# player4771/YOLO-DBL

Hardware: AMD Instinct MI355X
Metric: images/sec @640×640 bs=32 (1/2/4/8 GPU) + mAP@0.5 vs CPU ref (higher is better)
Workload: dtype fp16; 1 GPU; YOLO-DBL-n 640x640 bs=32/GPU fp16 forward+decode+NMS (conf .25, iou .7, max_det 300); model=yolov13n_DBL, global_batch=32, imgsz=640, nc=3, parallelism=dp1, streams_per_gpu=2

## Files before the change

### yolo-dbl_amd/csrc/conv.hip

```cpp
#include <stdlib.h>

#include "conv_common.hpp"

namespace ydbl {

template <bool Q8>
__device__ __forceinline__ int swz(int row, int kv) {
  if constexpr (Q8) return row * 4 + (kv ^ (((row >> 3) & 1) << 1));
  else return row * 4 + (kv ^ (((row >> 2) & 1) << 1));
}

template <typename T, int BM, int BN, int WM, int WN, bool POINTWISE, bool Q8, int PF = 1, int KA = ACT_RT>
__global__ __launch_bounds__(256) void conv_igemm_kernel(ConvArgs<T> p) {
  constexpr int VEC = Vec<T>::N;
  constexpr int BK = 4 * VEC;
  constexpr int TM = BM / WM / 16, TN = BN / WN / 16;
  static_assert(WM * WN == 4 && TM >= 1 && TN >= 1, "tile config");
  static_assert(PF >= 1 && PF <= 4, "prefetch depth");
  constexpr int A_IT = (BN * 4 + 255) / 256, B_IT = (BM * 4 + 255) / 256;
  using vec = typename Vec<T>::type;
  using opv = typename Op<T, Q8>::lds;
  __shared__ opv sA[2][BN * 4];
  __shared__ opv sB[2][BM * 4];

  const int tid = threadIdx.x;
  const int lane = tid & 63, wave = tid >> 6;
  const int g = lane >> 4, r16 = lane & 15;
  const int wm = wave % WM, wn = wave / WM;
  int mb, nb;
  xcd_tile2(mb, nb);
  const int m0 = mb * BM;
  const int n0 = nb * BN;
  __shared__ __align__(16) float s_bias[BN];
  BiasStage<BN> bst;
  bst.fetch(p.bias, n0, p.Cout);

  int64_t arow[A_IT];
  bool aval[A_IT];
#pragma unroll
  for (int it = 0; it < A_IT; ++it) {
    const int v = tid + it * 256;
    const int co = n0 + (v >> 2);
    aval[it] = v < BN * 4 && co < p.Cout;
    arow[it] = (int64_t)(aval[it] ? co : 0) * p.KPAD + (v & 3) * VEC;
  }
  int bb[B_IT], biy[B_IT], bix[B_IT];
  int64_t bpix[B_IT];
  bool bval[B_IT];
#pragma unroll
  for (int it = 0; it < B_IT; ++it) {
    const int v = tid + it * 256;
    int pp = m0 + (v >> 2);
    bval[it] = v < BM * 4 && pp < p.P;
    pp = bval[it] ? pp : 0;
    bpix[it] = pp;
    const int ox = pp % p.Wo;
    const int t = pp / p.Wo;
    const int oy = t % p.Ho;
    bb[it] = t / p.Ho;
    biy[it] = oy * p.S - p.PAD;
    bix[it] = ox * p.S - p.PAD;
  }
  opv ra[PF][A_IT];
  vec rb[PF][B_IT];
  bool rok[PF][B_IT], aok[PF][A_IT];
  int cur_ci = (tid & 3) * VEC, cur_kx = 0, cur_ky = 0;
  if constexpr (!POINTWISE) {
    const int tap = cur_ci / p.Cin;
    cur_ci -= tap * p.Cin;
    cur_ky = tap / p.KW;
    cur_kx = tap - cur_ky * p.KW;
  }
  auto advance = [&]() {
    if constexpr (!POINTWISE) {
      cur_ci += BK;
      while (cur_ci >= p.Cin) {
        cur_ci -= p.Cin;
        if (++cur_kx == p.KW) { cur_kx = 0; ++cur_ky; }
      }
    }
  };
  auto load_step = [&](int ks, opv (&a)[A_IT], bool (&aok)[A_IT], vec (&b)[B_IT], bool (&bok)[B_IT]) {
#pragma unroll
    for (int it = 0; it < A_IT; ++it) {
      aok[it] = aval[it] && ks * BK < p.KPAD;
      a[it] = load_wop_raw<T, Q8>(p.w, arow[it] + ks * BK, aok[it]);
    }
#pragma unroll
    for (int it = 0; it < B_IT; ++it) {
      const int v = tid + it * 256;
      const int k = ks * BK + (v & 3) * VEC;
      const bool kin = k < p.K;
      if constexpr (POINTWISE) {
        bok[it] = bval[it] && kin;
        b[it] = vload_clamped(p.x + bpix[it] * p.xcs + k, p.x, bok[it]);
      } else {
        const int iy = biy[it] + cur_ky * p.DIL, ix = bix[it] + cur_kx * p.DIL;
        bok[it] = bval[it] && kin && iy >= 0 && iy < p.H && ix >= 0 && ix < p.W;
        b[it] = vload_clamped(p.x + ((int64_t)(bb[it] * p.H + iy) * p.W + ix) * p.xcs + cur_ci, p.x, bok[it]);
      }
    }
    advance();
  };
  auto store_step = [&](int buf, const opv (&a)[A_IT], const bool (&aok)[A_IT], const vec (&b)[B_IT],
                        const bool (&bok)[B_IT]) {
#pragma unroll
    for (int it = 0; it < A_IT; ++it) {
      const int v = tid + it * 256;
      if (v < BN * 4) sA[buf][swz<Q8>(v >> 2, v & 3)] = vsel(a[it], aok[it]);
    }
#pragma unroll
    for (int it = 0; it < B_IT; ++it) {
      const int v = tid + it * 256;
      if (v < BM * 4) sB[buf][swz<Q8>(v >> 2, v & 3)] = to_op<T, Q8>(vsel(b[it], bok[it]), p.qs);
    }
  };

  f32x4 acc[TN][TM];
#pragma unroll
  for (int i = 0; i < TN; ++i)
#pragma unroll
    for (int j = 0; j < TM; ++j) acc[i][j] = f32x4{0.f, 0.f, 0.f, 0.f};

  const int nsteps = (p.K + BK - 1) / BK;
#pragma unroll
  for (int u = 0; u < PF; ++u) load_step(u, ra[u], aok[u], rb[u], rok[u]);
  store_step(0, ra[0], aok[0], rb[0], rok[0]);
  bst.commit(s_bias);
  __syncthreads();
  for (int k0 = 0; k0 < nsteps; k0 += PF) {
#pragma unroll
    for (int u = 0; u < PF; ++u) {
      const int ks = k0 + u;
      if (PF > 1 || ks + PF < nsteps) load_step(ks + PF, ra[u], aok[u], rb[u], rok[u]);
      if (ks < nsteps) {
        const int buf = ks & 1;
        opv af[TN], bf[TM];
#pragma unroll
        for (int i = 0; i < TN; ++i) af[i] = sA[buf][swz<Q8>(wn * TN * 16 + i * 16 + r16, g)];
#pragma unroll
        for (int j = 0; j < TM; ++j) bf[j] = sB[buf][swz<Q8>(wm * TM * 16 + j * 16 + r16, g)];
#pragma unroll
        for (int i = 0; i < TN; ++i)
#pragma unroll
          for (int j = 0; j < TM; ++j) acc[i][j] = mfma_op<T, Q8>(af[i], bf[j], acc[i][j]);
        const int nx = (u + 1) % PF;
        if (ks + 1 < nsteps) store_step(buf ^ 1, ra[nx], aok[nx], rb[nx], rok[nx]);
        __syncthreads();
      }
    }
  }

  int64_t pp[TM];
  bool pv[TM];
  int co[TN];
#pragma unroll
  for (int j = 0; j < TM; ++j) {
    pp[j] = m0 + wm * TM * 16 + j * 16 + r16;
    pv[j] = pp[j] < p.P;
  }
#pragma unroll
  for (int i = 0; i < TN; ++i) co[i] = n0 + wn * TN * 16 + i * 16 + 4 * g;
  conv_epilogue<T, TN, TM, Q8, KA>(p, acc, pp, pv, co, s_bias, n0);
}

template <int CV>
__device__ __forceinline__ int tswz(int pix, int cv) {
  if constexpr (CV == 1) return pix;
  else return pix * CV + (cv ^ ((pix / (16 / CV)) & (CV - 1)));
}

template <typename T, int CIN, int S, int TH, int TW, int NTN, int KA = ACT_RT>
__global__ __launch_bounds__(256) void conv3x3_tile_kernel(ConvArgs<T> p, int tiles_x, int tiles_y) {
  constexpr int VEC = Vec<T>::N;
  constexpr int CV = CIN / VEC;
  constexpr int IH = (TH - 1) * S + 3, IW = (TW - 1) * S + 3;
  constexpr int K = 9 * CIN;
  constexpr int BK = 4 * VEC;
  constexpr int KPAD = (K + 31) / 32 * 32;
  constexpr int NSTEP = (K + BK - 1) / BK;
  constexpr int WROW = KPAD / VEC + 1;
  constexpr int TM = TH * TW / 64;
  using vec = typename Vec<T>::type;
  __shared__ vec sx[IH * IW * CV];
  __shared__ vec sw[NTN * 16 * WROW];

  const int tid = threadIdx.x;
  int bid = xcd_remap(blockIdx.x, gridDim.x);
  const int tx = bid % tiles_x; bid /= tiles_x;
  const int ty = bid % tiles_y;
  const int b = bid / tiles_y;
  const int oy0 = ty * TH, ox0 = tx * TW;
  const int iy0 = oy0 * S - p.PAD, ix0 = ox0 * S - p.PAD;
  __shared__ __align__(16) float s_bias[NTN * 16];
  BiasStage<NTN * 16> bst;
  bst.fetch(p.bias, 0, p.Cout);
  {
    constexpr int TOT = IH * IW * CV;
    for (int base = 0; base < TOT; base += 4 * 256) {
      vec t[4];
#pragma unroll
      for (int u = 0; u < 4; ++u) {
        const int i = min(base + u * 256 + tid, TOT - 1);
        const int pix = i / CV, cv = i - pix * CV;
        const int iy = iy0 + pix / IW, ix = ix0 + pix % IW;
        const bool ok = iy >= 0 && iy < p.H && ix >= 0 && ix < p.W;
        t[u] = vload_sel(p.x + ((int64_t)(b * p.H + iy) * p.W + ix) * p.xcs + cv * VEC, p.x, ok);
      }
#pragma unroll
      for (int u = 0; u < 4; ++u) {
        const int i = base + u * 256 + tid;
        if (i < TOT) sx[tswz<CV>(i / CV, i % CV)] = t[u];
      }
    }
    constexpr int WTOT = NTN * 16 * (KPAD / VEC);
    for (int base = 0; base < WTOT; base += 4 * 256) {
      vec t[4];
#pragma unroll
      for (int u = 0; u < 4; ++u) {
        const int i = min(base + u * 256 + tid, WTOT - 1);
        const int co = i / (KPAD / VEC), kv = i % (KPAD / VEC);
        t[u] = vload_sel(p.w + (int64_t)co * p.KPAD + kv * VEC, p.w, co < p.Cout);
      }
#pragma unroll
      for (int u = 0; u < 4; ++u) {
        const int i = base + u * 256 + tid;
        if (i < WTOT) sw[(i / (KPAD / VEC)) * WROW + i % (KPAD / VEC)] = t[u];
      }
    }
  }
  bst.commit(s_bias);
  __syncthreads();

  const int lane = tid & 63, wave = tid >> 6;
  const int g = lane >> 4, r16 = lane & 15;
  int lbase[TM];
#pragma unroll
  for (int j = 0; j < TM; ++j) {
    const int op = wave * TM * 16 + j * 16 + r16;
    const int py = op / TW, px = op % TW;
    lbase[j] = (py * S) * IW + px * S;
  }
  f32x4 acc[NTN][TM];
#pragma unroll
  for (int i = 0; i < NTN; ++i)
#pragma unroll
    for (int j = 0; j < TM; ++j) acc[i][j] = f32x4{0.f, 0.f, 0.f, 0.f};
#pragma unroll
  for (int ks = 0; ks < NSTEP; ++ks) {
    const int k = ks * BK + g * VEC;
    const bool kin = k < K;
    const int tap = kin ? k / CIN : 0, cv = kin ? (k % CIN) / VEC : 0;
    const int ky = tap / 3, kx = tap % 3;
    const int toff = ky * IW + kx;
    vec af[NTN], bf[TM];
#pragma unroll
    for (int i = 0; i < NTN; ++i) af[i] = sw[(i * 16 + r16) * WROW + ks * 4 + g];
#pragma unroll
    for (int j = 0; j < TM; ++j) bf[j] = sx[tswz<CV>(lbase[j] + toff, cv)];
#pragma unroll
    for (int i = 0; i < NTN; ++i)
#pragma unroll
      for (int j = 0; j < TM; ++j) acc[i][j] = mfma_chunk<T>(af[i], bf[j], acc[i][j]);
  }

  int64_t pp[TM];
  bool pv[TM];
  int co[NTN];
#pragma unroll
  for (int j = 0; j < TM; ++j) {
    const int op = wave * TM * 16 + j * 16 + r16;
    const int oy = oy0 + op / TW, ox = ox0 + op % TW;
    pv[j] = oy < p.Ho && ox < p.Wo;
    pp[j] = ((int64_t)b * p.Ho + oy) * p.Wo + ox;
  }
#pragma unroll
  for (int i = 0; i < NTN; ++i) co[i] = i * 16 + 4 * g;
  conv_epilogue<T, NTN, TM, false, KA>(p, acc, pp, pv, co, s_bias, 0);
}

template <typename T, int CIN, int S, int TH, int TW, int NTN>
static void launch_tile(const ConvArgs<T>& a, hipStream_t s) {
  const int tiles_x = (int)cdiv(a.Wo, TW), tiles_y = (int)cdiv(a.Ho, TH);
  const unsigned grid = (unsigned)(a.N * tiles_y * tiles_x);
  if constexpr (sizeof(T) == 2) {
    const int form = epi_host_form(a);
    if (form == YDBL_ACT_SILU)
      return conv3x3_tile_kernel<T, CIN, S, TH, TW, NTN, YDBL_ACT_SILU><<<grid, 256, 0, s>>>(a, tiles_x, tiles_y);
    if (form == YDBL_ACT_NONE)
      return conv3x3_tile_kernel<T, CIN, S, TH, TW, NTN, YDBL_ACT_NONE><<<grid, 256, 0, s>>>(a, tiles_x, tiles_y);
  }
  conv3x3_tile_kernel<T, CIN, S, TH, TW, NTN, ACT_RT><<<grid, 256, 0, s>>>(a, tiles_x, tiles_y);
}

template <typename T, int CIN, int NTN>
static void launch_tile_s(const ConvArgs<T>& a, hipStream_t s) {
  if (a.S == 1) launch_tile<T, CIN, 1, 8, 32, NTN>(a, s);
  else launch_tile<T, CIN, 2, 8, 16, NTN>(a, s);
}

template <typename T, int CIN>
static bool tile_ntn(const ConvArgs<T>& a, hipStream_t s) {
  switch ((a.Cout + 15) / 16) {
    case 1: launch_tile_s<T, CIN, 1>(a, s); return true;
    case 2: launch_tile_s<T, CIN, 2>(a, s); return true;
    case 3: launch_tile_s<T, CIN, 3>(a, s); return true;
    case 4: launch_tile_s<T, CIN, 4>(a, s); return true;
    default: return false;
  }
}

template <typename T>
static bool try_tile(const ConvArgs<T>& a, int kh, hipStream_t s) {
  if (kh != 3 || a.KW != 3 || a.DIL != 1 || a.PAD != 1 || a.Cout > 64 || a.Cout % 4) return false;
  if (a.S != 1 && a.S != 2) return false;
  if ((int64_t)a.Ho * a.Wo < 4096) return false;
  if (a.xcs % Vec<T>::N) return false;
  switch (a.Cin) {
    case 8: return tile_ntn<T, 8>(a, s);
    case 16: return tile_ntn<T, 16>(a, s);
    case 32: return tile_ntn<T, 32>(a, s);
    default: return false;
  }
}

template <typename T, int BM, int BN, bool POINTWISE, bool Q8, int PF = 1, bool SPLIT = false>
__global__ __launch_bounds__(256) void conv_wsk_kernel(ConvArgs<T> p) {
  constexpr int VEC = Vec<T>::N;
  constexpr int BK = 4 * VEC;
  constexpr int BKB = 4 * BK;
  constexpr int TM = BM / 16, TN = BN / 16;
  constexpr int A_IT = BN * 16 / 256, B_IT = BM * 16 / 256;
  static_assert(A_IT >= 1 && B_IT >= 1, "tile");
  using vec = typename Vec<T>::type;
  using opv = typename Op<T, Q8>::lds;
  constexpr int STAGE = 2 * (BN + BM) * 16 * (int)sizeof(opv);
  constexpr int RED = 4 * TN * TM * 64 * 16;
  __shared__ f32x4 smem[(STAGE > RED ? STAGE : RED) / 16];
  opv* sA = reinterpret_cast<opv*>(smem);
  opv* sB = sA + 2 * BN * 16;

  const int tid = threadIdx.x;
  const int lane = tid & 63, wave = tid >> 6;
  const int g = lane >> 4, r16 = lane & 15;
  int mb, nb;
  xcd_tile2(mb, nb);
  const int m0 = mb * BM, n0 = nb * BN;
  const int kv = tid & 15;

  int64_t arow[A_IT];
  bool aval[A_IT];
#pragma unroll
  for (int it = 0; it < A_IT; ++it) {
    const int co = n0 + ((tid + it * 256) >> 4);
    aval[it] = co < p.Cout;
    arow[it] = (int64_t)(aval[it] ? co : 0) * p.KPAD + kv * VEC;
  }
  int bb[B_IT], biy[B_IT], bix[B_IT];
  int64_t bpix[B_IT];
  bool bval[B_IT];
#pragma unroll
  for (int it = 0; it < B_IT; ++it) {
    int pp = m0 + ((tid + it * 256) >> 4);
    bval[it] = pp < p.P;
    pp = bval[it] ? pp : 0;
    bpix[it] = pp;
    const int ox = pp % p.Wo;
    const int t = pp / p.Wo;
    bb[it] = t / p.Ho;
    biy[it] = (t % p.Ho) * p.S - p.PAD;
    bix[it] = ox * p.S - p.PAD;
  }
  const int nsteps_all = (p.K + BKB - 1) / BKB;
  const int z = SPLIT ? (int)blockIdx.z : 0;
  const int s0 = SPLIT ? (int)((int64_t)z * nsteps_all / p.ksplit) : 0;
  const int s1 = SPLIT ? (int)((int64_t)(z + 1) * nsteps_all / p.ksplit) : nsteps_all;
  int cur_ci = s0 * BKB + kv * VEC, cur_kx = 0, cur_ky = 0;
  if constexpr (!POINTWISE) {
    const int tap = cur_ci / p.Cin;
    cur_ci -= tap * p.Cin;
    cur_ky = tap / p.KW;
    cur_kx = tap - cur_ky * p.KW;
  }
  opv ra[PF][A_IT];
  vec rb[PF][B_IT];
  bool aok[PF], bok[PF][B_IT];
  auto load_step = [&](int kb, opv (&a)[A_IT], bool& ak, vec (&b)[B_IT], bool (&bk)[B_IT]) {
    const int k = kb * BKB + kv * VEC;
    const bool kin = k < p.K;
    ak = kin;
#pragma unroll
    for (int it = 0; it < A_IT; ++it) a[it] = load_wop_raw<T, Q8>(p.w, arow[it] + kb * BKB, aval[it] && kin);
#pragma unroll
    for (int it = 0; it < B_IT; ++it) {
      if constexpr (POINTWISE) {
        bk[it] = bval[it] && kin;
        b[it] = vload_clamped(p.x + bpix[it] * p.xcs + k, p.x, bk[it]);
      } else {
        const int iy = biy[it] + cur_ky * p.DIL, ix = bix[it] + cur_kx * p.DIL;
        bk[it] = bval[it] && kin && iy >= 0 && iy < p.H && ix >= 0 && ix < p.W;
        b[it] = vload_clamped(p.x + ((int64_t)(bb[it] * p.H + iy) * p.W + ix) * p.xcs + cur_ci, p.x, bk[it]);
      }
    }
    if constexpr (!POINTWISE) {
      cur_ci += BKB;
      while (cur_ci >= p.Cin) {
        cur_ci -= p.Cin;
        if (++cur_kx == p.KW) { cur_kx = 0; ++cur_ky; }
      }
    }
  };
  auto store_step = [&](int buf, const opv (&a)[A_IT], bool ak, const vec (&b)[B_IT], const bool (&bk)[B_IT]) {
#pragma unroll
    for (int it = 0; it < A_IT; ++it) {
      const int row = (tid + it * 256) >> 4;
      sA[buf * BN * 16 + row * 16 + (kv ^ (row & 15))] = vsel(a[it], aval[it] && ak);
    }
#pragma unroll
    for (int it = 0; it < B_IT; ++it) {
      const int row = (tid + it * 256) >> 4;
      sB[buf * BM * 16 + row * 16 + (kv ^ (row & 15))] = to_op<T, Q8>(vsel(b[it], bk[it]), p.qs);
    }
  };

  f32x4 acc[TN][TM];
#pragma unroll
  for (int i = 0; i < TN; ++i)
#pragma unroll
    for (int j = 0; j < TM; ++j) acc[i][j] = f32x4{0.f, 0.f, 0.f, 0.f};

  const int nsteps = s1 - s0;
#pragma unroll
  for (int u = 0; u < PF; ++u) load_step(s0 + u, ra[u], aok[u], rb[u], bok[u]);
  store_step(0, ra[0], aok[0], rb[0], bok[0]);
  __syncthreads();
  const int myk = wave * 4 + g;
  for (int k0 = 0; k0 < nsteps; k0 += PF) {
#pragma unroll
    for (int u = 0; u < PF; ++u) {
      const int kb = k0 + u;
      if (PF > 1 || kb + PF < nsteps) load_step(s0 + kb + PF, ra[u], aok[u], rb[u], bok[u]);
      if (kb < nsteps) {
        const int buf = kb & 1;
        opv af[TN], bf[TM];
#pragma unroll
        for (int i = 0; i < TN; ++i) {
          const int row = i * 16 + r16;
          af[i] = sA[buf * BN * 16 + row * 16 + (myk ^ (row & 15))];
        }
#pragma unroll
        for (int j = 0; j < TM; ++j) {
          const int row = j * 16 + r16;
          bf[j] = sB[buf * BM * 16 + row * 16 + (myk ^ (row & 15))];
        }
#pragma unroll
        for (int i = 0; i < TN; ++i)
#pragma unroll
          for (int j = 0; j < TM; ++j) acc[i][j] = mfma_op<T, Q8>(af[i], bf[j], acc[i][j]);
        const int nx = (u + 1) % PF;
        if (kb + 1 < nsteps) store_step(buf ^ 1, ra[nx], aok[nx], rb[nx], bok[nx]);
        __syncthreads();
      }
    }
  }

  f32x4* red = reinterpret_cast<f32x4*>(smem);
#pragma unroll
  for (int i = 0; i < TN; ++i)
#pragma unroll
    for (int j = 0; j < TM; ++j) red[((wave * TN + i) * TM + j) * 64 + lane] = acc[i][j];
  __syncthreads();
  for (int t = wave; t < TN * TM; t += 4) {
    const int i = t / TM, j = t % TM;
    f32x4 sum = red[((0 * TN + i) * TM + j) * 64 + lane];
#pragma unroll
    for (int w = 1; w < 4; ++w) {
      const f32x4 o = red[((w * TN + i) * TM + j) * 64 + lane];
      sum = f32x4{sum[0] + o[0], sum[1] + o[1], sum[2] + o[2], sum[3] + o[3]};
    }
    const f32x4 one[1][1] = {{sum}};
    const int64_t pp[1] = {m0 + j * 16 + r16};
    const bool pv[1] = {pp[0] < p.P};
    const int co[1] = {n0 + i * 16 + 4 * g};
    if constexpr (SPLIT) {
      if (pv[0] && co[0] < p.Cout)
        *reinterpret_cast<f32x4*>(p.ws + ((int64_t)z * p.P + pp[0]) * ((p.Cout + 3) & ~3) + co[0]) = sum;
    } else {
      conv_epilogue<T, 1, 1, Q8>(p, one, pp, pv, co);
    }
  }
}

template <typename T, bool Q8>
__global__ __launch_bounds__(256) void splitk_epilogue_kernel(ConvArgs<T> p) {
  const int c4 = (p.Cout + 3) >> 2, cs = c4 * 4;
  const int64_t t = (int64_t)blockIdx.x * 256 + threadIdx.x;
  const int64_t pix = t / c4;
  const int co = (int)(t - pix * c4) * 4;
  const bool ok = pix < p.P;
  const int64_t pc = ok ? pix : 0;
  f32x4 v[4];
#pragma unroll
  for (int z = 0; z < 4; ++z)
    v[z] = z < p.ksplit ? *reinterpret_cast<const f32x4*>(p.ws + ((int64_t)z * p.P + pc) * cs + co) : f32x4{0.f, 0.f, 0.f, 0.f};
  f32x4 sum = v[0];
#pragma unroll
  for (int z = 1; z < 4; ++z)
    if (z < p.ksplit) sum = f32x4{sum[0] + v[z][0], sum[1] + v[z][1], sum[2] + v[z][2], sum[3] + v[z][3]};
  const f32x4 one[1][1] = {{sum}};
  const int64_t pp[1] = {pix};
  const bool pv[1] = {ok};
  const int cc[1] = {co};
  conv_epilogue<T, 1, 1, Q8>(p, one, pp, pv, cc);
}

template <typename T, bool Q8>
void launch_splitk_epilogue(const ConvArgs<T>& a, hipStream_t s) {
  splitk_epilogue_kernel<T, Q8><<<(unsigned)cdiv((int64_t)a.P * ((a.Cout + 3) >> 2), 256), 256, 0, s>>>(a);
}
template void launch_splitk_epilogue<_Float16, false>(const ConvArgs<_Float16>&, hipStream_t);
template void launch_splitk_epilogue<_Float16, true>(const ConvArgs<_Float16>&, hipStream_t);
template void launch_splitk_epilogue<float, false>(const ConvArgs<float>&, hipStream_t);

constexpr int WSK_SPLIT_BELOW = 768;
template <typename T>
static int wsk_ksplit(const ConvArgs<T>& a, int bm, int bn) {
  const char* e = getenv("YDBL_SPLITK");
  if (sizeof(T) != 2 || (e && *e == '0')) return 1;
  const int64_t tiles = cdiv(a.P, bm) * cdiv(a.Cout, bn);
  const int nsteps = (int)cdiv(a.K, 16 * Vec<T>::N);
  if (tiles >= WSK_SPLIT_BELOW || nsteps < 16) return 1;
  int k = (int)std::min<int64_t>(4, (WSK_SPLIT_BELOW + tiles - 1) / tiles);
  while (k > 1 && nsteps / k < 8) --k;
  return k;
}
template <typename T>
static int64_t wsk_ws_bytes(const ConvArgs<T>& a, int ksplit) {
  return ksplit > 1 ? (int64_t)ksplit * a.P * ((a.Cout + 3) & ~3) * 4 : 0;
}

constexpr int WSK_PF = 2;

template <typename T, bool Q8, int BM, int BN>
static void launch_wsk(const ConvArgs<T>& a0, bool pointwise, hipStream_t s) {
  ConvArgs<T> a = a0;
  a.ksplit = wsk_ksplit(a, BM, BN);
  if (a.ksplit > 1 && (!a.ws || a.ws_bytes < wsk_ws_bytes(a, a.ksplit))) a.ksplit = 1;
  dim3 grid((unsigned)cdiv(a.P, BM), (unsigned)cdiv(a.Cout, BN), (unsigned)a.ksplit);
  if (a.ksplit > 1) {
    if (pointwise) conv_wsk_kernel<T, BM, BN, true, Q8, WSK_PF, true><<<grid, 256, 0, s>>>(a);
    else conv_wsk_kernel<T, BM, BN, false, Q8, WSK_PF, true><<<grid, 256, 0, s>>>(a);
    launch_splitk_epilogue<T, Q8>(a, s);
  } else if (pointwise) {
    conv_wsk_kernel<T, BM, BN, true, Q8, WSK_PF><<<grid, 256, 0, s>>>(a);
  } else {
    conv_wsk_kernel<T, BM, BN, false, Q8, WSK_PF><<<grid, 256, 0, s>>>(a);
  }
}

template <typename T>
static void wsk_tiles(const ConvArgs<T>& a, int& bm, int& bn) {
  auto blocks = [&](int m, int n) { return cdiv(a.P, m) * cdiv(a.Cout, n); };
  const int64_t want = 768;
  const char* eh = getenv("YDBL_WSK_HALF");
  if (a.Cout <= 128 && blocks(32, a.Cout <= 64 ? 64 : 128) < 256 && !(eh && *eh == '0')) {
    bm = a.Cout <= 64 ? 16 : 32;
    bn = 64;
    return;
  }
  if (a.Cout <= 32) { bm = blocks(128, 32) >= want ? 128 : 64; bn = 32; return; }
  if (a.Cout <= 64) { bm = blocks(64, 64) >= want ? 64 : 32; bn = 64; return; }
  bm = 32;
  bn = blocks(32, 128) >= want || a.Cout % 128 == 0 ? 128 : 64;
}

template <typename T>
static bool wsk_applies(const ConvArgs<T>& a) { return a.K >= 1024 || (a.K >= 512 && a.P <= 16384); }

template <typename T, bool Q8>
static bool try_wsk(const ConvArgs<T>& a, bool pointwise, hipStream_t s) {
  if (!wsk_applies(a)) return false;
  int bm, bn;
  wsk_tiles(a, bm, bn);
  if (bm == 16) launch_wsk<T, Q8, 16, 64>(a, pointwise, s);
  else if (bm == 32 && bn == 64) launch_wsk<T, Q8, 32, 64>(a, pointwise, s);
  else if (bm == 32) launch_wsk<T, Q8, 32, 128>(a, pointwise, s);
  else if (bm == 64 && bn == 64) launch_wsk<T, Q8, 64, 64>(a, pointwise, s);
  else if (bm == 64) launch_wsk<T, Q8, 64, 32>(a, pointwise, s);
  else launch_wsk<T, Q8, 128, 32>(a, pointwise, s);
  return true;
}

template <typename T, bool Q8, int BM, int BN, int WM, int WN>
static void launch_igemm(const ConvArgs<T>& a, bool pointwise, hipStream_t s) {
  dim3 grid((unsigned)cdiv(a.P, BM), (unsigned)cdiv(a.Cout, BN));
  if constexpr (sizeof(T) == 2 && !Q8) {
    const int form = pointwise ? epi_host_form(a) : ACT_RT;
    if (form == YDBL_ACT_SILU)
      return conv_igemm_kernel<T, BM, BN, WM, WN, true, Q8, 1, YDBL_ACT_SILU><<<grid, 256, 0, s>>>(a);
    if (form == YDBL_ACT_NONE)
      return conv_igemm_kernel<T, BM, BN, WM, WN, true, Q8, 1, YDBL_ACT_NONE><<<grid, 256, 0, s>>>(a);
  }
  if (pointwise)
    conv_igemm_kernel<T, BM, BN, WM, WN, true, Q8><<<grid, 256, 0, s>>>(a);
  else
    conv_igemm_kernel<T, BM, BN, WM, WN, false, Q8><<<grid, 256, 0, s>>>(a);
}

template <typename T, bool Q8>
static void dispatch_conv(const ConvArgs<T>& a, bool pointwise, hipStream_t s) {
  const int64_t want = a.Cout <= 128 && a.P <= 65536 ? 512
                       : (a.K <= 128 && a.P > (a.K <= 64 ? 65536 : 131072) ? 2048 : 1024);
  auto blocks = [&](int bm, int bn) { return cdiv(a.P, bm) * cdiv(a.Cout, bn); };
  if (a.Cout <= 16) {
    if (blocks(256, 16) >= want) return launch_igemm<T, Q8, 256, 16, 4, 1>(a, pointwise, s);
    if (blocks(128, 16) >= want) return launch_igemm<T, Q8, 128, 16, 4, 1>(a, pointwise, s);
    return launch_igemm<T, Q8, 64, 16, 4, 1>(a, pointwise, s);
  }
  if (a.Cout <= 32) {
    if (blocks(256, 32) >= want) return launch_igemm<T, Q8, 256, 32, 4, 1>(a, pointwise, s);
    if (blocks(128, 32) >= want) return launch_igemm<T, Q8, 128, 32, 4, 1>(a, pointwise, s);
    return launch_igemm<T, Q8, 64, 32, 4, 1>(a, pointwise, s);
  }
  if (a.Cout <= 64) {
    if (blocks(128, 64) >= want) return launch_igemm<T, Q8, 128, 64, 2, 2>(a, pointwise, s);
    if (blocks(64, 64) >= want || (!pointwise && a.K >= 512 && a.P >= 16384))
      return launch_igemm<T, Q8, 64, 64, 2, 2>(a, pointwise, s);
    return launch_igemm<T, Q8, 32, 64, 2, 2>(a, pointwise, s);
  }
  if (blocks(128, 64) >= want) return launch_igemm<T, Q8, 128, 64, 2, 2>(a, pointwise, s);
  if (blocks(64, 64) >= want) return launch_igemm<T, Q8, 64, 64, 2, 2>(a, pointwise, s);
  return launch_igemm<T, Q8, 32, 64, 2, 2>(a, pointwise, s);
}

template <typename T>
int halo_ksplit(const ConvArgs<T>& a, int64_t wgs);

template <typename T, bool Q8>
static void route(const ConvArgs<T>& a, int kh, bool pw, hipStream_t s) {
  if constexpr (sizeof(T) == 2 && !Q8) {
    if (try_conv3x3_vw(a, kh, s)) return;
  }
  if (!Q8 && try_tile<T>(a, kh, s)) return;
  if (try_conv3x3_halo<T, Q8>(a, kh, s)) return;
  if (try_wsk<T, Q8>(a, pw, s)) return;
  dispatch_conv<T, Q8>(a, pw, s);
}

template <typename T>
static ConvArgs<T> conv_args(const ydbl_conv_desc* d) {
  ConvArgs<T> a{};
  a.x = reinterpret_cast<const T*>(d->x.ptr);
  a.xcs = d->x.cs; a.N = d->x.n; a.H = d->x.h; a.W = d->x.w; a.Cin = d->x.c;
  a.y = reinterpret_cast<T*>(d->y.ptr);
  a.ycs = d->y.cs; a.Ho = d->y.h; a.Wo = d->y.w; a.Cout = d->y.c;
  a.r = reinterpret_cast<const T*>(d->r.ptr); a.rcs = d->r.cs;
  a.w = reinterpret_cast<const T*>(d->w); a.bias = d->bias;
  a.KW = d->kw; a.S = d->stride; a.PAD = d->pad; a.DIL = d->dil;
  a.K = d->kh * d->kw * d->x.c; a.KPAD = d->kpad;
  a.act = d->act; a.res = d->res_mode;
  a.epi_generic = epi_generic();
  a.P = d->y.n * d->y.h * d->y.w;
  a.y2 = reinterpret_cast<T*>(d->y2.ptr); a.y2cs = d->y2.cs;
  a.r2 = reinterpret_cast<const T*>(d->r2.ptr); a.r2cs = d->r2.cs;
  a.a2 = d->a2; a.b2 = d->b2;
  a.dq = d->dq; a.qs = d->qscale;
  a.ws = reinterpret_cast<float*>(d->workspace); a.ws_bytes = d->workspace ? d->workspace_bytes : 0;
  a.ksplit = 1;
  return a;
}

ConvArgs<_Float16> conv_args_f16(const ydbl_conv_desc* d) { return conv_args<_Float16>(d); }

template <typename T>
static int run_conv(const ydbl_conv_desc* d, hipStream_t s) {
  const ConvArgs<T> a = conv_args<T>(d);
  const bool pw = d->kh == 1 && d->kw == 1 && d->stride == 1 && d->pad == 0 && d->x.h == d->y.h && d->x.w == d->y.w;
  if constexpr (sizeof(T) == 2) {
    if (d->dq) {
      route<T, true>(a, d->kh, pw, s);
      return check_launch("ydbl_conv2d_nhwc");
    }
  }
  route<T, false>(a, d->kh, pw, s);
  return check_launch("ydbl_conv2d_nhwc");
}

int conv_check(const ydbl_conv_desc* d) {
  if (!d) return fail(YDBL_EINVAL, "conv: null descriptor");
  if (check_view(&d->x, "conv.x", true) || check_view(&d->y, "conv.y", false)) return YDBL_EINVAL;
  if (d->x.dtype != d->y.dtype) return fail(YDBL_EINVAL, "conv: x/y dtype mismatch");
  if (d->x.c % 8) return fail(YDBL_EINVAL, "conv: input channels must be a multiple of 8");
  if (d->x.n != d->y.n) return fail(YDBL_EINVAL, "conv: batch mismatch");
  if (d->kh < 1 || d->kw < 1 || d->stride < 1 || d->dil < 1 || d->pad < 0)
    return fail(YDBL_EINVAL, "conv: bad kernel geometry");
  const int ho = (d->x.h + 2 * d->pad - d->dil * (d->kh - 1) - 1) / d->stride + 1;
  const int wo = (d->x.w + 2 * d->pad - d->dil * (d->kw - 1) - 1) / d->stride + 1;
  if (ho != d->y.h || wo != d->y.w) return fail(YDBL_EINVAL, "conv: output spatial size mismatch");
  const int K = d->kh * d->kw * d->x.c;
  if (d->kpad < K || d->kpad % 32) return fail(YDBL_EINVAL, "conv: kpad must be >= K and a multiple of 32");
  if (!d->w) return fail(YDBL_EINVAL, "conv: null weights");
  if (d->y.cs % 4) return fail(YDBL_EINVAL, "conv: output channel stride must be a multiple of 4");
  if (d->res_mode != YDBL_RES_NONE) {
    if (check_view(&d->r, "conv.r", false)) return YDBL_EINVAL;
    if (d->r.cs % 4 || d->r.dtype != d->y.dtype) return fail(YDBL_EINVAL, "conv: residual stride/dtype");
    if (d->r.n != d->y.n || d->r.h != d->y.h || d->r.w != d->y.w || d->r.c < d->y.c)
      return fail(YDBL_EINVAL, "conv: residual shape mismatch");
  }
  if (d->dq && d->x.dtype != YDBL_F16) return fail(YDBL_EINVAL, "conv: fp8 operands need f16 activations");
  if (d->y2.ptr) {
    if (check_view(&d->y2, "conv.y2", false) || check_view(&d->r2, "conv.r2", false)) return YDBL_EINVAL;
    auto same = [&](const ydbl_view& v) {
      return v.n == d->y.n && v.h == d->y.h && v.w == d->y.w && v.c == d->y.c && v.dtype == d->y.dtype && v.cs % 4 == 0;
    };
    if (!same(d->y2) || !same(d->r2)) return fail(YDBL_EINVAL, "conv: y2/r2 must match y (shape, dtype, cs % 4)");
  }
  return YDBL_OK;
}

}

using namespace ydbl;

extern "C" int ydbl_conv2d_nhwc(const ydbl_conv_desc* d, void* stream) {
  if (const int rc = conv_check(d)) return rc;
  const hipStream_t s = as_stream(stream);
  return d->x.dtype == YDBL_F16 ? run_conv<_Float16>(d, s) : run_conv<float>(d, s);
}

template <typename T>
static int64_t conv_ws_t(const ydbl_conv_desc* d) {
  const ConvArgs<T> a = conv_args<T>(d);
  int64_t need = 0;
  if (wsk_applies(a)) {
    int bm, bn;
    wsk_tiles(a, bm, bn);
    need = wsk_ws_bytes(a, wsk_ksplit(a, bm, bn));
  }
  if (d->kh == 3 && d->kw == 3 && d->stride == 1 && d->pad == 1 && d->dil == 1 && (int64_t)a.P < 25600) {
    const int64_t wgs = (int64_t)a.N * cdiv(a.Ho, 8) * cdiv(a.Wo, 16) * cdiv(a.Cout, 32);
    need = std::max(need, wsk_ws_bytes(a, halo_ksplit(a, wgs)));
  }
  return need;
}
extern "C" int64_t ydbl_conv_workspace(const ydbl_conv_desc* d) {
  if (conv_check(d)) return -1;
  return d->x.dtype == YDBL_F16 ? conv_ws_t<_Float16>(d) : conv_ws_t<float>(d);
}
```

### yolo-dbl_amd/ydbl/runtime.py

```python

from __future__ import annotations

import ctypes as C
import operator
import os
import time
from dataclasses import dataclass, field

import torch

from . import _lib
from ._lib import View, lib


SWITCHES = ("YDBL_DS2_OFF", "YDBL_DS_LEAN", "YDBL_HG_UNFUSED", "YDBL_HALO_NB", "YDBL_HALO_SMALL", "YDBL_VW", "YDBL_WSK_HALF",
            "YDBL_LSK_FUSE", "YDBL_NMS_FAST", "YDBL_NMS_GROUPS", "YDBL_SPLITK", "YDBL_NO_BNECK", "YDBL_NO_BOX3",
            "YDBL_NO_CLS_TAIL", "YDBL_DWPW", "YDBL_NO_PAIR3", "YDBL_NO_FUSE_PAD", "YDBL_NO_MERGE", "YDBL_NO_STEM2",
            "YDBL_EPI_GENERIC", "YDBL_NO_SPARSE_BOX", "YDBL_NO_HG_PAIR")


def ydbl_env() -> tuple:
    get = os.environ.get
    return tuple(get(k) for k in SWITCHES)


_STRUCT_EPOCH = [0]


def _bump_epoch(*_):
    _STRUCT_EPOCH[0] += 1


for _reg in ("register_module_parameter_registration_hook", "register_module_buffer_registration_hook",
             "register_module_module_registration_hook"):
    getattr(torch.nn.modules.module, _reg)(_bump_epoch)
_VERSION = operator.attrgetter("_version")


def weights_signature(module: torch.nn.Module) -> tuple:
    c = module.__dict__.get("_wsig_cache")
    if c is None or c[0] != _STRUCT_EPOCH[0]:
        ts = [t for t in (*module.parameters(), *module.buffers()) if t.is_floating_point()]
        c = (_STRUCT_EPOCH[0], ts, hash(tuple((id(t), t.data_ptr()) for t in ts)))
        module.__dict__["_wsig_cache"] = c
    return c[2], sum(map(_VERSION, c[1]))


def round_up(x: int, m: int) -> int:
    return (x + m - 1) // m * m


class TV:

    __slots__ = ("base", "off", "n", "h", "w", "c", "cs")

    def __init__(self, base: torch.Tensor, off: int, n: int, h: int, w: int, c: int, cs: int):
        self.base, self.off, self.n, self.h, self.w, self.c, self.cs = base, off, n, h, w, c, cs

    @property
    def dtype(self):
        return self.base.dtype

    @property
    def ptr(self) -> int:
        return self.base.data_ptr() + self.off * self.base.element_size()

    @property
    def shape(self):
        return (self.n, self.h, self.w, self.c)

    def cslice(self, c0: int, c: int) -> "TV":
        assert 0 <= c0 and c0 + c <= self.c, (c0, c, self.c)
        return TV(self.base, self.off + c0, self.n, self.h, self.w, c, self.cs)

    def with_hw(self, h: int, w: int) -> "TV":
        assert h * w == self.h * self.w
        return TV(self.base, self.off, self.n, h, w, self.c, self.cs)

    def struct(self) -> View:
        return View(self.ptr, self.n, self.h, self.w, self.c, self.cs, _lib.dtype_code(self.dtype))

    def torch(self) -> torch.Tensor:
        return torch.as_strided(
            self.base, (self.n, self.h, self.w, self.c), (self.h * self.w * self.cs, self.w * self.cs, self.cs, 1),
            self.off,
        )

    def nchw(self) -> torch.Tensor:
        return self.torch().permute(0, 3, 1, 2)


@dataclass
class Step:
    fn: object
    args: tuple
    what: str
    keep: list = field(default_factory=list)


class Plan:

    def __init__(self, device: torch.device, dtype: torch.dtype):
        self.device = torch.device(device)
        self.dtype = dtype
        self.steps: list[Step] = []
        self.buffers: list[torch.Tensor] = []
        self.bytes_allocated = 0
        self._writers: dict = {}
        self.fp8_candidates: list = []
        self.fp8_layers: list = []

    def alloc(self, n: int, h: int, w: int, c: int, dtype: torch.dtype | None = None, cs: int | None = None) -> TV:
        dtype = dtype or self.dtype
        cs = cs or round_up(c, 8)
        t = torch.empty(n * h * w * cs, dtype=dtype, device=self.device)
        self.buffers.append(t)
        self.bytes_allocated += t.numel() * t.element_size()
        return TV(t, 0, n, h, w, c, cs)

    def scratch(self, nbytes: int, zero: bool = False) -> torch.Tensor:
        t = (torch.zeros if zero else torch.empty)(max(int(nbytes), 16), dtype=torch.uint8, device=self.device)
        self.buffers.append(t)
        self.bytes_allocated += t.numel()
        return t

    def splitk_scratch(self, nbytes: int) -> torch.Tensor:
        cur = getattr(self, "_splitk", None)
        if cur is None or cur.numel() < nbytes:
            cur = self._splitk = self.scratch(nbytes)
        return cur

    def const(self, t: torch.Tensor) -> torch.Tensor:
        t = t.detach().to(self.device).contiguous()
        self.buffers.append(t)
        return t

    def launch(self, name: str, *args, what: str = "", keep=()):
        self.steps.append(Step(getattr(lib, name), args, what or name, list(keep)))

    @staticmethod
    def _vkey(v: TV):
        return (v.base.data_ptr(), v.off, v.n, v.h, v.w, v.c, v.cs)

    def note_writer(self, y: TV, desc) -> None:
        self._writers[self._vkey(y)] = (len(self.steps) - 1, desc)

    def writer_of(self, v: TV):
        return self._writers.get(self._vkey(v))

    def made_before(self, v: TV, step: int) -> bool:
        w = self.writer_of(v)
        return w is not None and w[0] < step

    def fuse_second_output(self, writer, y2: TV, r2: TV, a2: float, b2: float) -> TV | None:
        _, d = writer
        if not hasattr(d, "y2") or d.y2.ptr:
            return None
        y = d.y
        for v in (y2, r2):
            if (v.n, v.h, v.w, v.c) != (y.n, y.h, y.w, y.c) or _lib.dtype_code(v.dtype) != y.dtype or v.cs % 4:
                return None
            if isinstance(d, (_lib.DySampleDesc, _lib.DySample2Desc)):
                vec = 16 // v.base.element_size()
                if v.cs % vec or v.c % vec or v.ptr % 16:
                    return None
        d.y2, d.r2, d.a2, d.b2 = y2.struct(), r2.struct(), float(a2), float(b2)
        self.steps[writer[0]].keep.append((y2, r2))
        return y2

    def check_single_stream(self):
        for st in self.steps:
            if not (isinstance(st.fn, C._CFuncPtr) or getattr(st.fn, "single_stream", False)):
                raise RuntimeError(f"plan step '{st.what}' ({st.fn!r}) is not a single-stream launch: it cannot be "
                                   f"captured as a branch of a split session's graph")

    def run_observed(self, observe, stream: int | None = None):
        s = C.c_void_p(torch.cuda.current_stream(self.device).cuda_stream if stream is None else stream)
        for i, st in enumerate(self.steps):
            observe(i)
            rc = st.fn(*st.args, s)
            if rc:
                _lib.check(rc, st.what)

    def run(self, stream: int | None = None):
        s = C.c_void_p(torch.cuda.current_stream(self.device).cuda_stream if stream is None else stream)
        for st in self.steps:
            rc = st.fn(*st.args, s)
            if rc:
                _lib.check(rc, st.what)

    def run_timed(self):
        stream = torch.cuda.current_stream(self.device)
        s = C.c_void_p(stream.cuda_stream)
        evs = []
        torch.cuda._sleep(int(1e8))
        for st in self.steps:
            a = torch.cuda.Event(enable_timing=True)
            b = torch.cuda.Event(enable_timing=True)
            a.record(stream)
            rc = st.fn(*st.args, s)
            b.record(stream)
            if rc:
                _lib.check(rc, st.what)
            evs.append((st.what, a, b))
        torch.cuda.synchronize(self.device)
        return [(w, a.elapsed_time(b)) for w, a, b in evs]

    def run_graph_timed(self, reps: int = 8, iters: int = 3):
        out = []
        for st in self.steps:
            self.run()
            g = torch.cuda.CUDAGraph()
            with torch.cuda.graph(g):
                s = C.c_void_p(torch.cuda.current_stream(self.device).cuda_stream)
                for _ in range(reps):
                    rc = st.fn(*st.args, s)
                    if rc:
                        _lib.check(rc, st.what)
            g.replay()
            torch.cuda.synchronize(self.device)
            a = torch.cuda.Event(enable_timing=True)
            b = torch.cuda.Event(enable_timing=True)
            best = float("inf")
            for _ in range(iters):
                torch.cuda._sleep(int(2e6))
                a.record()
                g.replay()
                b.record()
                torch.cuda.synchronize(self.device)
                best = min(best, a.elapsed_time(b) / reps)
            out.append((st.what, best))
            del g
        return out


class GraphRunner:

    def __init__(self, plan: Plan, warmup: int = 1, pre: Plan | None = None):
        self.plan = plan
        side = torch.cuda.Stream(plan.device)
        side.wait_stream(torch.cuda.current_stream(plan.device))
        with torch.cuda.stream(side):
            for _ in range(warmup):
                if pre is not None:
                    pre.run(side.cuda_stream)
                plan.run(side.cuda_stream)
        torch.cuda.current_stream(plan.device).wait_stream(side)
        torch.cuda.synchronize(plan.device)
        self.graph = torch.cuda.CUDAGraph()
        with torch.cuda.graph(self.graph):
            if pre is not None:
                pre.run()
            plan.run()
        torch.cuda.synchronize(plan.device)

    def replay(self):
        self.graph.replay()


class BranchGraphRunner:

    def __init__(self, plans, warmup: int = 1, pre: Plan | None = None):
        for p in plans:
            p.check_single_stream()
        dev = plans[0].device
        side = torch.cuda.Stream(dev)
        side.wait_stream(torch.cuda.current_stream(dev))
        with torch.cuda.stream(side):
            for _ in range(warmup):
                if pre is not None:
                    pre.run(side.cuda_stream)
                for p in plans:
                    p.run(side.cuda_stream)
        torch.cuda.current_stream(dev).wait_stream(side)
        torch.cuda.synchronize(dev)
        self.sides = [torch.cuda.Stream(dev) for _ in plans[1:]]
        self.graph = torch.cuda.CUDAGraph()
        with torch.cuda.graph(self.graph):
            cap = torch.cuda.current_stream(dev)
            if pre is not None:
                pre.run()
            for st in self.sides:
                st.wait_stream(cap)
            plans[0].run()
            for p, st in zip(plans[1:], self.sides):
                with torch.cuda.stream(st):
                    p.run(st.cuda_stream)
            for st in self.sides:
                cap.wait_stream(st)
        torch.cuda.synchronize(dev)

    def replay(self):
        self.graph.replay()


def timed(fn, *a, sync_device=None, **k):
    t0 = time.perf_counter()
    r = fn(*a, **k)
    if sync_device is not None:
        torch.cuda.synchronize(sync_device)
    return r, time.perf_counter() - t0
```

Measured before the change: 19260 images/s.

## Add specialized thin-channel 3x3 conv kernel with register-resident weights

Adds a dedicated 3x3 convolution kernel for a few small channel shapes (16->32 s2, 32->64 s2/s1). Each workgroup stages a spatial input tile with halo into LDS, keeps the full weight slice in registers, and computes with 16x16x32 fp16 MFMA over taps, followed by the shared epilogue. It is routed ahead of the generic tile/halo/igemm paths to cut im2col-style overhead and weight reloads on the early high-resolution layers. Adds an env switch to disable it, and the extra register pressure may lower occupancy.

New measurement: 19400 images/s (median of 6 runs). About the same (+0.8%).

```diff
diff --git a/yolo-dbl_amd/csrc/conv.hip b/yolo-dbl_amd/csrc/conv.hip
--- a/yolo-dbl_amd/csrc/conv.hip
+++ b/yolo-dbl_amd/csrc/conv.hip
@@ -635,11 +635,13 @@
 
 template <typename T>
 int halo_ksplit(const ConvArgs<T>& a, int64_t wgs);
+bool try_conv3x3_thin(const ConvArgs<_Float16>& a, int kh, hipStream_t s);
 
 template <typename T, bool Q8>
 static void route(const ConvArgs<T>& a, int kh, bool pw, hipStream_t s) {
   if constexpr (sizeof(T) == 2 && !Q8) {
     if (try_conv3x3_vw(a, kh, s)) return;
+    if (try_conv3x3_thin(a, kh, s)) return;
   }
   if (!Q8 && try_tile<T>(a, kh, s)) return;
   if (try_conv3x3_halo<T, Q8>(a, kh, s)) return;
diff --git a/yolo-dbl_amd/csrc/conv3x3_thin.hip b/yolo-dbl_amd/csrc/conv3x3_thin.hip
--- /dev/null
+++ b/yolo-dbl_amd/csrc/conv3x3_thin.hip
@@ -0,0 +1,134 @@
+#include <stdlib.h>
+
+#include "conv_common.hpp"
+
+namespace ydbl {
+
+template <int CIN, int S, int NT, int ROWS, int KA, int MW>
+__global__ __launch_bounds__(256, MW) void conv3x3_thin_kernel(ConvArgs<_Float16> p, int tiles_x, int tiles_y) {
+  constexpr int CH = CIN / 8, KS = (9 * CIN + 31) / 32;
+  constexpr int TPW = 1, NWG = NT / TPW, RW = 4 / NWG;
+  constexpr int TH = 8, TW = S == 1 ? 32 : 16;
+  constexpr int IH = (TH - 1) * S + 3, IW = (TW - 1) * S + 3, NPX = IH * IW;
+  constexpr int PIN = S == 1 ? (NPX + 15) / 16 * 16 : (NPX | 1);
+  constexpr int PT = TH * TW / 16 / RW;
+  static_assert((CH == 2 || CH == 4) && NT % TPW == 0 && 4 % NWG == 0 && PT % ROWS == 0, "conv3x3_thin shape");
+  __shared__ __align__(16) unsigned char s_in[CH * PIN * 16];
+  __shared__ __align__(16) float s_bias[NT * 16];
+
+  const int tid = threadIdx.x, lane = tid & 63, wave = wave_id();
+  const int g = lane >> 4, r16 = lane & 15;
+  int bid = xcd_remap(blockIdx.x, gridDim.x);
+  const int tx = bid % tiles_x; bid /= tiles_x;
+  const int ty = bid % tiles_y;
+  const int img = bid / tiles_y;
+  const int oy0 = ty * TH, ox0 = tx * TW;
+  const int iy0 = oy0 * S - 1, ix0 = ox0 * S - 1;
+  BiasStage<NT * 16> bst;
+  bst.fetch(p.bias, 0, p.Cout);
+
+  constexpr int PXU = 256 / CH, IT = (NPX + PXU - 1) / PXU;
+  const int s_chunk = (tid >> 3) % CH, px0 = ((tid >> 3) / CH) * 8 + (tid & 7);
+  h8 xr[IT];
+#pragma unroll
+  for (int u = 0; u < IT; ++u) {
+    const int px = px0 + u * PXU;
+    const int r = px / IW, c = px - r * IW;
+    const int iy = iy0 + r, ix = ix0 + c;
+    const bool ok = px < NPX && iy >= 0 && iy < p.H && ix >= 0 && ix < p.W;
+    const _Float16* src = ok ? p.x + ((int64_t)(img * p.H + iy) * p.W + ix) * p.xcs + s_chunk * 8 : p.x;
+    const h8 v = *reinterpret_cast<const h8*>(src);
+    xr[u] = ok ? v : h8{0, 0, 0, 0, 0, 0, 0, 0};
+  }
+  const int cg = wave % NWG;
+  h8 a[TPW][KS];
+#pragma unroll
+  for (int tt = 0; tt < TPW; ++tt) {
+    const _Float16* wrow = p.w + (int64_t)((cg * TPW + tt) * 16 + r16) * p.KPAD + g * 8;
+#pragma unroll
+    for (int m = 0; m < KS; ++m) a[tt][m] = *reinterpret_cast<const h8*>(wrow + 32 * m);
+  }
+  unsigned char* s_dst = s_in + (s_chunk * PIN + px0) * 16;
+#pragma unroll
+  for (int u = 0; u < IT; ++u)
+    if (px0 + u * PXU < NPX) *reinterpret_cast<h8*>(s_dst + u * PXU * 16) = xr[u];
+  bst.commit(s_bias);
+  __syncthreads();
+
+  int co[TPW];
+#pragma unroll
+  for (int tt = 0; tt < TPW; ++tt) co[tt] = (cg * TPW + tt) * 16 + 4 * g;
+  int ko[KS];
+#pragma unroll
+  for (int m = 0; m < KS; ++m) {
+    if constexpr (CH == 4) {
+      ko[m] = (g * PIN + (m / 3) * IW + m % 3) * 16;
+    } else {
+      const int tap = 2 * m + (g >> 1);
+      const bool kin = tap < 9;
+      ko[m] = kin ? ((g & 1) * PIN + (tap / 3) * IW + tap % 3) * 16 : 0;
+    }
+  }
+
+  ConvArgs<_Float16> pe = p;
+  pe.bias = nullptr;
+
+#pragma nounroll
+  for (int q0 = (wave / NWG) * PT; q0 < (wave / NWG + 1) * PT; q0 += ROWS) {
+    const unsigned char* in_b[ROWS];
+    int64_t pp[ROWS];
+    bool pv[ROWS];
+#pragma unroll
+    for (int r = 0; r < ROWS; ++r) {
+      const int q = q0 + r;
+      const int py = q / (TW / 16), px = (q % (TW / 16)) * 16 + r16;
+      in_b[r] = s_in + ((py * S) * IW + px * S) * 16;
+      const int oy = oy0 + py, ox = ox0 + px;
+      pv[r] = oy < p.Ho && ox < p.Wo;
+      pp[r] = ((int64_t)img * p.Ho + oy) * p.Wo + ox;
+    }
+    f32x4 acc[TPW][ROWS];
+#pragma unroll
+    for (int tt = 0; tt < TPW; ++tt)
+#pragma unroll
+      for (int r = 0; r < ROWS; ++r) acc[tt][r] = f32x4{0.f, 0.f, 0.f, 0.f};
+#pragma unroll
+    for (int m = 0; m < KS; ++m) {
+      h8 bf[ROWS];
+#pragma unroll
+      for (int r = 0; r < ROWS; ++r) bf[r] = *reinterpret_cast<const h8*>(in_b[r] + ko[m]);
+#pragma unroll
+      for (int r = 0; r < ROWS; ++r)
+#pragma unroll
+        for (int tt = 0; tt < TPW; ++tt)
+          acc[tt][r] = __builtin_amdgcn_mfma_f32_16x16x32_f16(a[tt][m], bf[r], acc[tt][r], 0, 0, 0);
+    }
+    conv_epilogue<_Float16, TPW, ROWS, false, KA>(pe, acc, pp, pv, co, s_bias, 0);
+  }
+}
+
+template <int CIN, int S, int NT, int ROWS, int ROWS_RT = ROWS, int MW_RT = 4>
+static void launch_thin(const ConvArgs<_Float16>& a, hipStream_t s) {
+  constexpr int TW = S == 1 ? 32 : 16;
+  const int tiles_x = (int)cdiv(a.Wo, TW), tiles_y = (int)cdiv(a.Ho, 8);
+  const unsigned grid = (unsigned)(a.N * tiles_y * tiles_x);
+  const int form = epi_host_form(a);
+  if (form == YDBL_ACT_SILU)
+    return conv3x3_thin_kernel<CIN, S, NT, ROWS, YDBL_ACT_SILU, 4><<<grid, 256, 0, s>>>(a, tiles_x, tiles_y);
+  if (form == YDBL_ACT_NONE)
+    return conv3x3_thin_kernel<CIN, S, NT, ROWS, YDBL_ACT_NONE, 4><<<grid, 256, 0, s>>>(a, tiles_x, tiles_y);
+  conv3x3_thin_kernel<CIN, S, NT, ROWS_RT, ACT_RT, MW_RT><<<grid, 256, 0, s>>>(a, tiles_x, tiles_y);
+}
+
+bool try_conv3x3_thin(const ConvArgs<_Float16>& a, int kh, hipStream_t s) {
+  if (kh != 3 || a.KW != 3 || a.DIL != 1 || a.PAD != 1) return false;
+  if ((int64_t)a.Ho * a.Wo < 4096 || a.xcs % 8) return false;
+  const char* e = getenv("YDBL_THIN3");
+  if (e && *e == '0') return false;
+  if (a.Cin == 16 && a.Cout == 32 && a.S == 2) return launch_thin<16, 2, 2, 2>(a, s), true;
+  if (a.Cin == 32 && a.Cout == 64 && a.S == 2) return launch_thin<32, 2, 4, 4, 2>(a, s), true;
+  if (a.Cin == 32 && a.Cout == 64 && a.S == 1) return launch_thin<32, 1, 4, 4, 4, 1>(a, s), true;
+  return false;
+}
+
+}
diff --git a/yolo-dbl_amd/ydbl/runtime.py b/yolo-dbl_amd/ydbl/runtime.py
--- a/yolo-dbl_amd/ydbl/runtime.py
+++ b/yolo-dbl_amd/ydbl/runtime.py
@@ -16,7 +16,7 @@
 SWITCHES = ("YDBL_DS2_OFF", "YDBL_DS_LEAN", "YDBL_HG_UNFUSED", "YDBL_HALO_NB", "YDBL_HALO_SMALL", "YDBL_VW", "YDBL_WSK_HALF",
             "YDBL_LSK_FUSE", "YDBL_NMS_FAST", "YDBL_NMS_GROUPS", "YDBL_SPLITK", "YDBL_NO_BNECK", "YDBL_NO_BOX3",
             "YDBL_NO_CLS_TAIL", "YDBL_DWPW", "YDBL_NO_PAIR3", "YDBL_NO_FUSE_PAD", "YDBL_NO_MERGE", "YDBL_NO_STEM2",
-            "YDBL_EPI_GENERIC", "YDBL_NO_SPARSE_BOX", "YDBL_NO_HG_PAIR")
+            "YDBL_EPI_GENERIC", "YDBL_NO_SPARSE_BOX", "YDBL_NO_HG_PAIR", "YDBL_THIN3")
 
 
 def ydbl_env() -> tuple:
```
